# jstrom2002/Mini-OpenCL-Raytracer

Measured on AMD Instinct MI355X. Metric: Mrays/s (3840x2160 Cornell box, 8 spp, 9 bounces), higher is better.
Workload: dtype f32

## Files before the change

### include/rt_hip.h

```cpp
#ifndef RT_HIP_H
#define RT_HIP_H

#include <stddef.h>
#include <stdint.h>

#include "rt_cl_types.h"
#include "rt_status.h"

#ifdef __cplusplus
extern "C" {
#endif

typedef struct rt_context_s* rt_context;
typedef struct rt_mem_s* rt_mem;
typedef struct rt_kernel_s* rt_kernel;

#define RT_MEM_READ_WRITE (1u << 0)
#define RT_MEM_WRITE_ONLY (1u << 1)
#define RT_MEM_READ_ONLY (1u << 2)
#define RT_MEM_COPY_HOST_PTR (1u << 5)

enum rt_kernel_arg {
    RT_ARG_BUFFER_OUT = 0,
    RT_ARG_BUFFER_SCENE = 1,
// ... 68 lines not shown
    uint64_t launches;
    double kernel_ms;
    uint64_t cycles_refill, cycles_traverse, cycles_shade, cycles_total;
    uint64_t sched[12];
    double accum_ms;
    double render_period_ms;
} rt_stats;
int rtKernelSetStats(rt_kernel k, int enable);
int rtKernelSetTiming(rt_kernel k, int enable);
int rtKernelGetStats(rt_kernel k, rt_stats* out);
int rtKernelResetStats(rt_kernel k);

typedef struct rt_path_kill_info {
    uint64_t zero_hits, zero_misses;
    int32_t scene_certified, launch_certified;
} rt_path_kill_info;
int rtKernelGetPathKill(rt_kernel k, rt_path_kill_info* out);

typedef struct rt_node_collapse_info {
    uint32_t collapsed_links;
    int32_t scene_collapsible, launch_collapsed;
} rt_node_collapse_info;
int rtKernelGetNodeCollapse(rt_kernel k, rt_node_collapse_info* out);

typedef struct rt_ray {
    float origin[3];
    float tmin;
    float dir[3];
    float tmax;
} rt_ray;
typedef struct rt_ray_hit {
    int32_t prim;
    float t, u, v;
} rt_ray_hit;
#define RT_QUERY_CLOSEST 0
#define RT_QUERY_ANY 1
int rtEnqueueIntersectRays(rt_context ctx, rt_kernel k, rt_mem rays, size_t first_ray, size_t n_rays, int mode,
                           rt_mem hits);
int rtEnqueueCameraRays(rt_context ctx, rt_kernel k, size_t global_work_size, rt_mem rays);

typedef struct rt_path_result {
    float radiance[3];
    int32_t prim;
} rt_path_result;
#define RT_TRACE_LINEAR 0
#define RT_TRACE_FRAME0 1
// ... 232 lines not shown
```

### mini-opencl-raytracer_amd/clrt/_native.py

```python
from __future__ import annotations

import ctypes
import os

import numpy as np

_PKG_ROOT = os.path.dirname(os.path.dirname(os.path.abspath(__file__)))
LIB_DIR = os.path.join(_PKG_ROOT, "lib")
HIP_LIB_PATH = os.environ.get("RT_HIP_LIB") or os.path.join(LIB_DIR, "librt_hip.so")
SCENE_LIB_PATH = os.path.join(LIB_DIR, "librt_scene.so")

RT_SUCCESS = 0
_ERROR_NAMES = {
    0: "CL_SUCCESS", -1: "CL_DEVICE_NOT_FOUND", -4: "CL_MEM_OBJECT_ALLOCATION_FAILURE",
    -5: "CL_OUT_OF_RESOURCES", -6: "CL_OUT_OF_HOST_MEMORY", -30: "CL_INVALID_VALUE",
    -33: "CL_INVALID_DEVICE", -34: "CL_INVALID_CONTEXT", -36: "CL_INVALID_COMMAND_QUEUE",
    -37: "CL_INVALID_HOST_PTR", -38: "CL_INVALID_MEM_OBJECT", -46: "CL_INVALID_KERNEL_NAME",
    -48: "CL_INVALID_KERNEL", -49: "CL_INVALID_ARG_INDEX", -50: "CL_INVALID_ARG_VALUE",
    -51: "CL_INVALID_ARG_SIZE", -52: "CL_INVALID_KERNEL_ARGS", -59: "CL_INVALID_OPERATION",
    -61: "CL_INVALID_BUFFER_SIZE", -63: "CL_INVALID_GLOBAL_WORK_SIZE",
    -1001: "RT_FILE_NOT_FOUND", -1002: "RT_PARSE_ERROR",
}


# ... 69 lines not shown
          "step_weight_leaf_global": 25, "query_refill_min": 26}
TRACE_TUNING = {"trace_refill_min": 28, "trace_shade_min": 29}
PATH_KILL_TUNING = {"path_kill": 30}


class Stats(ctypes.Structure):
    _fields_ = [("rays", ctypes.c_uint64), ("node_visits", ctypes.c_uint64),
                ("tri_tests", ctypes.c_uint64), ("hits", ctypes.c_uint64),
                ("launches", ctypes.c_uint64), ("kernel_ms", ctypes.c_double),
                ("cycles_refill", ctypes.c_uint64), ("cycles_traverse", ctypes.c_uint64),
                ("cycles_shade", ctypes.c_uint64), ("cycles_total", ctypes.c_uint64),
                ("sched", ctypes.c_uint64 * 12), ("accum_ms", ctypes.c_double),
                ("render_period_ms", ctypes.c_double)]


class PathKillInfo(ctypes.Structure):
    _fields_ = [("zero_hits", ctypes.c_uint64), ("zero_misses", ctypes.c_uint64),
                ("scene_certified", ctypes.c_int32), ("launch_certified", ctypes.c_int32)]


class NodeCollapseInfo(ctypes.Structure):
    _fields_ = [("collapsed_links", ctypes.c_uint32), ("scene_collapsible", ctypes.c_int32),
                ("launch_collapsed", ctypes.c_int32)]


class TRACE_PARAMS(ctypes.Structure):
    _fields_ = [("seed_base", ctypes.c_uint32), ("encoding", ctypes.c_int)]


class ADAPTIVE_PARAMS(ctypes.Structure):
    _fields_ = [("threshold", ctypes.c_float), ("floor_y", ctypes.c_float), ("min_samples", ctypes.c_uint32),
                ("max_samples", ctypes.c_uint32), ("radius", ctypes.c_uint32)]


class DENOISE_PARAMS(ctypes.Structure):
    _fields_ = [("iterations", ctypes.c_uint), ("sigma_color", ctypes.c_float), ("sigma_normal", ctypes.c_float),
                ("sigma_depth", ctypes.c_float), ("sigma_albedo", ctypes.c_float)]


class DENOISE_SAMPLES_PARAMS(ctypes.Structure):
    _fields_ = [("iterations", ctypes.c_uint), ("sigma_luminance", ctypes.c_float), ("sigma_normal", ctypes.c_float),
                ("sigma_depth", ctypes.c_float), ("sigma_albedo", ctypes.c_float), ("epsilon", ctypes.c_float),
                ("encoding", ctypes.c_int)]


DENOISE_LINEAR, DENOISE_GAMMA = 0, 1
# ... 85 lines not shown
                                          ctypes.c_size_t, _vp]),
    "rtEnqueueFrameMotion": (ctypes.c_int, [_vp, _vp, ctypes.c_size_t, _vp, _vp, ctypes.c_size_t, ctypes.c_size_t, _vp]),
    "rtRefitBVH": (ctypes.c_int, [_vp, _vp]),
    "rtDiagScenePrepares": (ctypes.c_int, [_vp, ctypes.POINTER(ctypes.c_uint64), ctypes.POINTER(ctypes.c_uint64)]),
    "rtEnqueueReadBuffer": (ctypes.c_int, [_vp, _vp, ctypes.c_int, ctypes.c_size_t, ctypes.c_size_t, _vp]),
    "rtEnqueueWriteBuffer": (ctypes.c_int, [_vp, _vp, ctypes.c_int, ctypes.c_size_t, ctypes.c_size_t, _vp]),
    "rtFinish": (ctypes.c_int, [_vp]),
    "rtEnqueueCopyBufferToPointer": (ctypes.c_int, [_vp, _vp, ctypes.c_size_t, ctypes.c_size_t, _vp]),
    "rtKernelSetMathMode": (ctypes.c_int, [_vp, ctypes.c_int]),
    "rtKernelSetWorkRange": (ctypes.c_int, [_vp, ctypes.c_uint64, ctypes.c_uint64]),
    "rtKernelSetSchedule": (ctypes.c_int, [_vp, ctypes.c_int]),
    "rtKernelSetRowInterleave": (ctypes.c_int, [_vp, ctypes.c_uint, ctypes.c_uint]),
    "rtEnqueueCopyBufferRectToPointer": (ctypes.c_int, [_vp, _vp, ctypes.c_size_t, ctypes.c_size_t, ctypes.c_size_t,
                                                        ctypes.c_size_t, _vp, ctypes.c_size_t]),
    "rtEnqueueCopyPointerRectToBuffer": (ctypes.c_int, [_vp, _vp, ctypes.c_size_t, _vp, ctypes.c_size_t,
                                                        ctypes.c_size_t, ctypes.c_size_t, ctypes.c_size_t]),
    "rtKernelSetHitBuffers": (ctypes.c_int, [_vp, _vp, _vp]),
    "rtKernelSetStats": (ctypes.c_int, [_vp, ctypes.c_int]),
    "rtKernelSetTiming": (ctypes.c_int, [_vp, ctypes.c_int]),
    "rtKernelGetStats": (ctypes.c_int, [_vp, ctypes.POINTER(Stats)]),
    "rtKernelResetStats": (ctypes.c_int, [_vp]),
    "rtKernelGetPathKill": (ctypes.c_int, [_vp, ctypes.POINTER(PathKillInfo)]),
    "rtKernelGetNodeCollapse": (ctypes.c_int, [_vp, ctypes.POINTER(NodeCollapseInfo)]),
    "rtKernelGetSceneInLDS": (ctypes.c_int, [_vp, ctypes.POINTER(ctypes.c_int)]),
    "rtKernelForceGlobalScene": (ctypes.c_int, [_vp, ctypes.c_int]),
    "rtBuildBVH": (ctypes.c_int, [_vp, _vp, ctypes.c_size_t, ctypes.c_uint, _vp, ctypes.POINTER(ctypes.c_size_t)]),
    "rtBuildBVHEx": (ctypes.c_int, [_vp, _vp, ctypes.c_size_t, ctypes.c_uint, ctypes.c_int, _vp,
                                    ctypes.POINTER(ctypes.c_size_t)]),
    "rtBufferGetDevicePointer": (ctypes.c_int, [_vp, ctypes.POINTER(_vp)]),
    "rtBufferGetSize": (ctypes.c_int, [_vp, ctypes.POINTER(ctypes.c_size_t)]),
    "rtContextGetStream": (ctypes.c_int, [_vp, ctypes.POINTER(_vp)]),
    "rtContextSetReadbackOnAccumStream": (ctypes.c_int, [_vp, ctypes.c_int]),
    "rtContextGetAccumStream": (ctypes.c_int, [_vp, ctypes.POINTER(_vp)]),
    "rtContextGetDevice": (ctypes.c_int, [_vp, ctypes.POINTER(ctypes.c_int)]),
    "rtValidateBVH": (ctypes.c_int, [_vp, ctypes.c_size_t, ctypes.c_size_t, ctypes.POINTER(ctypes.c_int)]),
    "rtKernelSetTuning": (ctypes.c_int, [_vp, ctypes.c_int, ctypes.c_int]),
    "rtKernelGetTuning": (ctypes.c_int, [_vp, ctypes.c_int, ctypes.POINTER(ctypes.c_int)]),
    "rtContextSetAccumOverlap": (ctypes.c_int, [_vp, ctypes.c_int]),
    "rtCommGetUniqueId": (ctypes.c_int, [_vp]),
    "rtCommInitRank": (ctypes.c_int, [_vp, ctypes.c_int, _vp, ctypes.c_int, ctypes.POINTER(_vp)]),
    "rtCommInitAll": (ctypes.c_int, [ctypes.POINTER(_vp), ctypes.c_int, ctypes.POINTER(_vp)]),
    "rtCommInitLoopback": (ctypes.c_int, [ctypes.POINTER(_vp), ctypes.c_int, ctypes.POINTER(_vp)]),
    "rtCommInitShared": (ctypes.c_int, [_vp, ctypes.c_int, ctypes.c_int, ctypes.c_char_p, ctypes.POINTER(_vp)]),
    "rtCommDestroy": (ctypes.c_int, [_vp]),
    "rtCommGetRank": (ctypes.c_int, [_vp, ctypes.POINTER(ctypes.c_int), ctypes.POINTER(ctypes.c_int)]),
    "rtCommShardKernel": (ctypes.c_int, [_vp, _vp]),
# ... 80 lines not shown
```

### mini-opencl-raytracer_amd/clrt/device.py

```python
from __future__ import annotations

import ctypes
import struct

import numpy as np

from . import _native as N
from ._native import RTError, check, hip_lib


def _tuning_id(name: str) -> int:
    for table in (N.TUNING, N.TRACE_TUNING):
        if name in table:
            return table[name]
    return N.PATH_KILL_TUNING[name]


class CLContext:

    def __init__(self, device: int = 0):
        self._lib = hip_lib()
        h = ctypes.c_void_p()
        check(self._lib.rtCreateContext(int(device), ctypes.byref(h)), "Failed to create context")
        self.handle = h
# ... 331 lines not shown
        sched = dict(zip(("node_steps", "node_lanes", "tri_steps", "tri_lanes", "shade_rounds",
                          "shade_lanes", "refill_rounds", "refill_lanes", "other_lanes",
                          "shade_wait", "free_wait", "reserved"), list(s.sched)))
        sched["refill_pops"] = sched["reserved"]
        return {"rays": s.rays, "node_visits": s.node_visits, "tri_tests": s.tri_tests,
                "hits": s.hits, "launches": s.launches, "kernel_ms": s.kernel_ms, "accum_ms": s.accum_ms,
                "render_period_ms": s.render_period_ms,
                "cycles": {"refill": s.cycles_refill, "traverse": s.cycles_traverse,
                           "shade": s.cycles_shade, "total": s.cycles_total},
                "sched": sched}

    def path_kill(self) -> dict:
        s = N.PathKillInfo()
        check(self._lib.rtKernelGetPathKill(self.handle, ctypes.byref(s)), "path kill")
        return {"zero_hits": int(s.zero_hits), "zero_misses": int(s.zero_misses),
                "scene_certified": bool(s.scene_certified), "launch_certified": bool(s.launch_certified)}

    def node_collapse(self) -> dict:
        s = N.NodeCollapseInfo()
        check(self._lib.rtKernelGetNodeCollapse(self.handle, ctypes.byref(s)), "node collapse")
        return {"collapsed_links": int(s.collapsed_links), "scene_collapsible": bool(s.scene_collapsible),
                "launch_collapsed": bool(s.launch_collapsed)}

    def scene_prepares(self) -> tuple:
        full, refits = ctypes.c_uint64(), ctypes.c_uint64()
        check(self._lib.rtDiagScenePrepares(self.handle, ctypes.byref(full), ctypes.byref(refits)),
              "scene prepares")
        return int(full.value), int(refits.value)

    def reset_stats(self) -> None:
        check(self._lib.rtKernelResetStats(self.handle), "reset stats")

    def release(self) -> None:
        if self.handle:
            self._lib.rtReleaseKernel(self.handle)
            self.handle = None
```

### mini-opencl-raytracer_amd/csrc/rt_capi.cpp

```cpp
#include <hip/hip_runtime.h>

#include <algorithm>
#include <limits>
#include <cstdlib>
#include <cstring>
#include <mutex>
#include <new>
#include <vector>

#include "../../include/rt_cl_types.h"
#include "../../include/rt_hip.h"
#include "rt_adaptive.hpp"
#include "rt_adaptive_plan.hpp"
#include "rt_bvh.hpp"
#include "rt_denoise.hpp"
#include "rt_denoise_plan.hpp"
#include "rt_denoise_samples.hpp"
#include "rt_device_scene.hpp"
#include "rt_internal.hpp"
#include "rt_kernel_state.hpp"
#include "rt_kernels.hpp"
#include "rt_launch_plan.hpp"
#include "rt_motion_launch.hpp"
#include "rt_motion_plan.hpp"
#include "rt_query_plan.hpp"
#include "rt_refit.hpp"
#include "rt_reproject.hpp"
#include "rt_reproject_plan.hpp"
#include "rt_scene_pack.hpp"
#include "rt_temporal.hpp"
#include "rt_temporal_plan.hpp"
#include "rt_trace_plan.hpp"
#include "rt_tuning.hpp"

namespace {

constexpr uint64_t kKnownFlags =
    RT_MEM_READ_WRITE | RT_MEM_WRITE_ONLY | RT_MEM_READ_ONLY | RT_MEM_COPY_HOST_PTR;
#ifndef RT_TIMELINE
#define RT_TIMELINE 0
#endif
constexpr size_t kHitPad = RT_TIMELINE ? 192 : 0;
#ifndef RT_NODE_COLLAPSE_STATS
#define RT_NODE_COLLAPSE_STATS 0
#endif

}

using rti::map_hip;
using rti::mark_device_write;
using rti::qs;

struct rt_kernel_s {
    rt_context ctx = nullptr;
    rti::LaunchArgs args;
    int math = RT_MATH_SHIPPED;
    int sched = RT_SCHED_STEP;
    rtp::Tuning tune;
    uint32_t band_period = 1, band_phase = 0;
    uint64_t range_first = 0, range_last = 0;
    bool comm_sharded = false;
    rt_mem hit_ids = nullptr, hit_t = nullptr;
    bool stats = false, timing = false, force_global = false;
    uint64_t launches = 0;
    uint64_t pf_waits = ~0ull;
    bool last_lds = false;
    bool last_kill = false;
    bool last_collapsed = false;
    rti::DeviceScene scene;
    rti::LaunchTimer timer;
    rti::RadianceSets rad;
    rti::WavefrontQueues wfq;
    rti::WorkCounters counters;
    rti::FeatureScratch feat;
    rti::DenoiseScratch denoise;
    rti::AdaptiveScratch adaptive;
    rtk::OccupancyCache occ;

    void release_parts() {
        timer.release();
        rad.release();
        wfq.release();
        counters.release();
        scene.release();
        feat.release();
        denoise.release();
        adaptive.release();
    }
};

namespace {
// ... 334 lines not shown
    in.light_bounces = la.light_bounces();
    in.gws = global_work_size;
    in.range_first = k->range_first, in.range_last = k->range_last;
    in.n_frames = n_frames;
    in.sched = k->sched, in.math = k->math;
    in.stats = k->stats, in.hit_bound = k->hit_ids != nullptr;
    in.fused = fused, in.overlap = ctx->overlap;
    in.band_period = k->band_period, in.band_phase = k->band_phase;
    const rti::DeviceScene& sc = k->scene;
    in.n_nodes = sc.n_nodes(), in.n_tris = sc.n_tris(), in.n_mats = sc.n_mats(), in.n_top = sc.n_top();
    in.oct_ok = sc.oct_ok();
    in.goct_available = sc.goct() != nullptr, in.goct_b = sc.goct_b();
    in.force_global = k->force_global;
    in.tune = k->tune;
    in.num_cus = ctx->num_cus;
    if (const float* rb = sc.root_bounds()) in.view = rtp::view_cull_rect(in.W, in.H, la.f3[0], la.f3[1], la.f3[2], rb, rb + 3);
    in.kill_scene_ok = sc.path_kill_ok(k->math == RT_MATH_SHIPPED);
    in.light_type = la.light_type(), in.skybox_intensity = la.skybox_intensity();
    return in;
}

static const float4* oct_records(rt_kernel k, rtk::Walk w, bool regrouped) {
    const rti::DeviceScene& sc = k->scene;
    const bool collapsed = sc.collapse_ok() && (!k->stats || RT_NODE_COLLAPSE_STATS);
    k->last_collapsed = collapsed && w != rtk::Walk::GlobalNodes;
    if (collapsed) return regrouped ? sc.goct_collapsed() : sc.oct_nodes_collapsed();
    return regrouped ? sc.goct() : sc.oct_nodes();
}

static void fill_args(rt_kernel k, const LaunchArgs& la, uint32_t first_frame, const rtp::LaunchPlan& p,
                      rtk::KernelArgs* args) {
    rtk::KernelArgs& a = *args;
    std::memset(&a, 0, sizeof(a));
    a.result = static_cast<float4*>(la.out()->dptr);
    a.trisFull = static_cast<const rt_cl_triangle*>(la.tris()->dptr);
    a.materials = static_cast<const rt_cl_material*>(la.materials()->dptr);
    const rti::DeviceScene& sc = k->scene;
    a.packedTris = sc.packed_tris();
    a.octNodes = oct_records(k, p.variant.walk, p.regrouped);
    a.gNodes = sc.g_nodes();
    a.shadeTris = sc.shade_tris();
    a.shadeMats = sc.shade_mats() + (k->math == RT_MATH_SHIPPED ? 4 * (size_t)sc.n_mats() : 0);
    a.nMats = sc.n_mats(), a.nTris = sc.n_tris();
    a.nNodes = p.nNodes, a.octStride = p.octStride, a.octB = p.octB, a.octRecords = p.octRecords, a.nTop = p.nTop;
    fill_camera(la, first_frame, &a);
    a.lightBounces = la.light_bounces(), a.lightType = la.light_type();
    a.skyboxIntensity = la.skybox_intensity();
    a.gidBegin = p.gidBegin, a.gidEnd = p.gidEnd;
// ... 1144 lines not shown
    int rc = ensure_device(k->ctx);
    if (rc) return rc;
    unsigned long long h[2] = {};
    hipError_t e = hipMemcpyAsync(h, k->counters.stats() + rti::WorkCounters::kZeroBetaWord, sizeof(h),
                                  hipMemcpyDeviceToHost, qs(k->ctx));
    if (e == hipSuccess) e = hipStreamSynchronize(qs(k->ctx));
    if (e != hipSuccess) return map_hip(e);
    out->zero_hits = h[0];
    out->zero_misses = h[1];
    out->scene_certified = k->scene.path_kill_ok(k->math == RT_MATH_SHIPPED) ? 1 : 0;
    out->launch_certified = k->last_kill ? 1 : 0;
    return RT_SUCCESS;
}

int rtKernelGetNodeCollapse(rt_kernel k, rt_node_collapse_info* out) {
    if (!k || !out) return RT_INVALID_VALUE;
    flush_kernel(k);
    out->collapsed_links = k->scene.collapsed_links();
    out->scene_collapsible = k->scene.collapse_ok() ? 1 : 0;
    out->launch_collapsed = k->last_collapsed ? 1 : 0;
    return RT_SUCCESS;
}

int rtKernelResetStats(rt_kernel k) {
    if (!k) return RT_INVALID_KERNEL;
    flush_kernel(k);
    int rc = ensure_device(k->ctx);
    if (rc) return rc;
    rc = k->timer.drain();
    if (rc) return rc;
    k->launches = 0;
    k->timer.reset();
    hipError_t e = k->counters.zero_stats(qs(k->ctx));
    if (e == hipSuccess) e = hipStreamSynchronize(qs(k->ctx));
    return map_hip(e);
}

int rtKernelGetSceneInLDS(rt_kernel k, int* in_lds) {
    if (!k || !in_lds) return RT_INVALID_VALUE;
    *in_lds = k->last_lds ? 1 : 0;
    return RT_SUCCESS;
}

int rtKernelForceGlobalScene(rt_kernel k, int force) {
    if (!k) return RT_INVALID_KERNEL;
    flush_kernel(k);
// ... 104 lines not shown
```

### mini-opencl-raytracer_amd/csrc/rt_device_scene.cpp

```cpp
#include "rt_device_scene.hpp"

#include <cstring>
#include <vector>

#include "rt_kernels.hpp"
#include "rt_path_kill.hpp"
#include "rt_refit.hpp"
#include "rt_scene_pack.hpp"

namespace rti {

namespace {

int host_bytes(rt_mem m, std::vector<uint8_t>& tmp, const uint8_t** out) {
    if (m->shadow_valid) {
        *out = m->shadow.data();
        return RT_SUCCESS;
    }
    tmp.resize(m->size);
    hipError_t e = hipMemcpyAsync(tmp.data(), m->dptr, m->size, hipMemcpyDeviceToHost, qs(m->ctx));
    if (e == hipSuccess) e = hipStreamSynchronize(qs(m->ctx));
    if (e != hipSuccess) return map_hip(e);
    *out = tmp.data();
    return RT_SUCCESS;
}

template <class T>
int ensure_dev(T*& p, size_t& cap, size_t count) {
    if (cap >= count) return RT_SUCCESS;
    if (p) (void)hipFree(p);
    p = nullptr;
    cap = 0;
    hipError_t e = hipMalloc(&p, count * sizeof(T));
    if (e != hipSuccess) return map_hip(e);
    cap = count;
    return RT_SUCCESS;
}

hipError_t upload(void* dst, const std::vector<uint32_t>& src, hipStream_t st) {
    return hipMemcpyAsync(dst, src.data(), src.size() * sizeof(uint32_t), hipMemcpyHostToDevice, st);
}

}

int DeviceScene::allocate(uint32_t nn, uint32_t nt, uint32_t nmat, size_t goct_words, bool collapsed) {
    int rc = ensure_dev(g_nodes_, g_nodes_cap_, (size_t)nn * 4);
    if (!rc) rc = ensure_dev(refit_links_, refit_links_cap_, (size_t)nn * 2);
    if (!rc) rc = ensure_dev(refit_arrivals_, refit_arrivals_cap_, (size_t)nn);
    if (!rc) rc = ensure_dev(oct_nodes_, oct_nodes_cap_, (size_t)rtp::oct_records(nn));
    if (!rc) rc = ensure_dev(goct_nodes_, goct_nodes_cap_, goct_words / 4);
    if (!rc && collapsed) rc = ensure_dev(oct_collapsed_, oct_collapsed_cap_, (size_t)rtp::oct_records(nn));
    if (!rc && collapsed) rc = ensure_dev(goct_collapsed_, goct_collapsed_cap_, goct_words / 4);
    if (!rc) rc = ensure_dev(packed_tris_, packed_tris_cap_, (size_t)nt * 3);
    if (!rc) rc = ensure_dev(shade_tris_, shade_tris_cap_, (size_t)nt * 3);
    if (!rc) rc = ensure_dev(shade_mats_, shade_mats_cap_, (size_t)nmat * 8);
    return rc;
}

int DeviceScene::prepare(rt_context ctx, rt_mem tm, rt_mem nm, rt_mem mm) {
    if (!stale(tm, nm, mm)) return RT_SUCCESS;
    std::vector<uint8_t> tmp_t, tmp_n;
    rtp::SceneBytes in;
    in.tris_size = tm->size, in.nodes_size = nm->size;
    int rc = host_bytes(tm, tmp_t, &in.tris);
    if (!rc) rc = host_bytes(nm, tmp_n, &in.nodes);
    if (rc) return rc;
    if (mm) {
        in.mats = static_cast<const uint8_t*>(mm->dptr);
        in.mats_size = mm->size;
    }
    rtp::HostPack p;
    rc = rtp::pack_scene_host(in, top_limit, &p);
    if (rc) return rc;
    invalidate();
    rc = allocate(p.n_nodes, p.n_tris, p.n_mats, p.goct_nodes.size(), p.collapsed_links != 0);
    if (rc) return rc;
    hipStream_t st = qs(ctx);
    hipError_t e = upload(g_nodes_, p.global_nodes, st);
    if (e == hipSuccess) e = upload(refit_links_, p.refit_links, st);
    if (e == hipSuccess) e = upload(oct_nodes_, p.oct_nodes, st);
    if (e == hipSuccess && !p.goct_nodes.empty()) e = upload(goct_nodes_, p.goct_nodes, st);
    if (e == hipSuccess && p.collapsed_links) e = upload(oct_collapsed_, p.oct_nodes_collapsed, st);
    if (e == hipSuccess && !p.goct_nodes_collapsed.empty()) e = upload(goct_collapsed_, p.goct_nodes_collapsed, st);
    if (e == hipSuccess)
        e = rtk::launch_pack(static_cast<const rt_cl_triangle*>(tm->dptr), p.n_tris, packed_tris_, shade_tris_,
                             mm ? static_cast<const rt_cl_material*>(mm->dptr) : nullptr, p.n_mats, shade_mats_, st);
    const hipError_t waited = hipStreamSynchronize(st);
    if (e == hipSuccess) e = waited;
    if (e != hipSuccess) return map_hip(e);
    n_nodes_ = p.n_nodes, n_tris_ = p.n_tris, n_mats_ = p.n_mats, n_top_ = p.n_top;
    oct_ok_ = p.oct_ok, goct_b_ = p.goct_b;
    collapsed_links_ = p.collapsed_links, collapse_known_ = RT_NODE_COLLAPSE != 0;
    root_known_ = p.n_nodes > 0 && in.nodes_size >= sizeof(rt_cl_bvh_node);
    if (root_known_) {
        rt_cl_bvh_node root;
        std::memcpy(&root, in.nodes, sizeof(root));
        const float b[6] = {root.bounds.pmin.x, root.bounds.pmin.y, root.bounds.pmin.z,
                            root.bounds.pmax.x, root.bounds.pmax.y, root.bounds.pmax.z};
        std::memcpy(root_bounds_, b, sizeof(b));
    }
    kill_known_ = false;
    if (mm && p.n_mats > 0) {
        std::vector<float> recs((size_t)p.n_mats * 32);
        e = hipMemcpyAsync(recs.data(), shade_mats_, recs.size() * sizeof(float), hipMemcpyDeviceToHost, st);
        if (e == hipSuccess) e = hipStreamSynchronize(st);
        if (e != hipSuccess) return map_hip(e);
        const rt_cl_triangle* ht = reinterpret_cast<const rt_cl_triangle*>(in.tris);
        for (int t = 0; t < 2; ++t)
            kill_ok_[t] = rtp::path_kill_scene_ok(recs.data() + (size_t)t * 16 * p.n_mats, p.n_mats, ht, p.n_tris,
                                                  root_bounds());
        kill_known_ = true;
    }
    for_tris_ = tm, tris_gen_ = tm->generation, tris_struct_ = tm->structural;
    for_nodes_ = nm, nodes_gen_ = nm->generation, nodes_struct_ = nm->structural;
    for_mats_ = mm, mats_gen_ = mm ? mm->generation : 0;
// ... 2 lines not shown
}

int DeviceScene::refit(rt_context ctx, rt_mem tm, rt_mem nm, rt_mem mm) {
    if (!structurally_current(tm, nm)) {
        invalidate();
        const int rc = prepare(ctx, tm, nm, mm);
        if (rc) return rc;
    }
    rtr::RefitArgs a{};
    a.tris = static_cast<const rt_cl_triangle*>(tm->dptr);
    a.n_tris = n_tris_;
    a.nodes = static_cast<rt_cl_bvh_node*>(nm->dptr);
    a.n_nodes = n_nodes_;
    a.parent = refit_links_;
    a.slot = refit_links_ + n_nodes_;
    a.arrivals = refit_arrivals_;
    a.oct = oct_nodes_;
    a.oct_stride = rtp::oct_stride(n_nodes_), a.oct_b = rtp::oct_b(n_nodes_);
    a.goct = goct_b_ ? goct_nodes_ : nullptr;
    a.goct_b = goct_b_, a.goct_group = RT_GOCT_GROUP ? RT_GOCT_GROUP : 1;
    a.g_nodes = g_nodes_;
    root_known_ = false;
    collapse_known_ = false;
    kill_known_ = false;
    hipStream_t st = qs(ctx);
    hipError_t e = rtr::launch_refit(a, st);
    if (e == hipSuccess) e = rtk::launch_pack(a.tris, n_tris_, packed_tris_, shade_tris_, nullptr, 0, shade_mats_, st);
    mark_device_write(nm, false);
    if (e != hipSuccess) {
        invalidate();
        return map_hip(e);
    }
    tris_gen_ = tm->generation;
    nodes_gen_ = nm->generation;
    ++refits_;
    return RT_SUCCESS;
}

void DeviceScene::release() {
    for (void* p : {(void*)packed_tris_, (void*)shade_tris_, (void*)shade_mats_, (void*)oct_nodes_, (void*)goct_nodes_,
                    (void*)oct_collapsed_, (void*)goct_collapsed_, (void*)g_nodes_, (void*)refit_links_,
                    (void*)refit_arrivals_})
        if (p) (void)hipFree(p);
    *this = DeviceScene();
}

}
```

### mini-opencl-raytracer_amd/csrc/rt_device_scene.hpp

```cpp
#pragma once

#include <hip/hip_runtime.h>
#include <stdint.h>

#include "rt_internal.hpp"

namespace rti {

class DeviceScene {
public:
    uint32_t top_limit = 384;

    int prepare(rt_context ctx, rt_mem tris, rt_mem nodes, rt_mem mats);
    int refit(rt_context ctx, rt_mem tris, rt_mem nodes, rt_mem mats);
    void invalidate() { for_nodes_ = nullptr; }
    void release();

    uint32_t n_nodes() const { return n_nodes_; }
    uint32_t n_tris() const { return n_tris_; }
    uint32_t n_mats() const { return n_mats_; }
    uint32_t n_top() const { return n_top_; }
    bool oct_ok() const { return oct_ok_; }
    uint32_t goct_b() const { return goct_b_; }
    const float4* packed_tris() const { return packed_tris_; }
    const float4* shade_tris() const { return shade_tris_; }
    const float4* shade_mats() const { return shade_mats_; }
    const float4* oct_nodes() const { return oct_nodes_; }
    const float4* g_nodes() const { return g_nodes_; }
    const float4* goct() const { return goct_b_ ? goct_nodes_ : nullptr; }
    bool collapse_ok() const { return collapse_known_; }
    uint32_t collapsed_links() const { return collapsed_links_; }
    const float4* oct_nodes_collapsed() const { return collapsed_links_ ? oct_collapsed_ : oct_nodes_; }
    const float4* goct_collapsed() const { return collapsed_links_ && goct_b_ ? goct_collapsed_ : goct(); }
    const float* root_bounds() const { return root_known_ ? root_bounds_ : nullptr; }
    bool path_kill_ok(bool shipped) const { return kill_known_ && kill_ok_[shipped ? 1 : 0]; }
    uint64_t full_prepares() const { return full_prepares_; }
    uint64_t refits() const { return refits_; }

private:
    bool stale(rt_mem tris, rt_mem nodes, rt_mem mats) const {
        return for_tris_ != tris || tris_gen_ != tris->generation || for_nodes_ != nodes ||
               nodes_gen_ != nodes->generation || (mats && (for_mats_ != mats || mats_gen_ != mats->generation));
    }
    bool structurally_current(rt_mem tris, rt_mem nodes) const {
        return for_tris_ == tris && for_nodes_ == nodes && tris_struct_ == tris->structural &&
               nodes_struct_ == nodes->structural;
    }
    int allocate(uint32_t n_nodes, uint32_t n_tris, uint32_t n_mats, size_t goct_words, bool collapsed);

    rt_mem for_tris_ = nullptr, for_nodes_ = nullptr, for_mats_ = nullptr;
    uint64_t tris_gen_ = 0, nodes_gen_ = 0, mats_gen_ = 0;
    uint64_t tris_struct_ = 0, nodes_struct_ = 0;
    uint32_t n_nodes_ = 0, n_tris_ = 0, n_mats_ = 0, n_top_ = 0, goct_b_ = 0;
    bool oct_ok_ = false;
    bool root_known_ = false;
    float root_bounds_[6] = {};
    bool collapse_known_ = false;
    uint32_t collapsed_links_ = 0;
    bool kill_known_ = false;
    bool kill_ok_[2] = {false, false};
    uint64_t full_prepares_ = 0, refits_ = 0;
    float4 *packed_tris_ = nullptr, *shade_tris_ = nullptr, *shade_mats_ = nullptr;
    float4 *oct_nodes_ = nullptr, *goct_nodes_ = nullptr, *g_nodes_ = nullptr;
    size_t packed_tris_cap_ = 0, shade_tris_cap_ = 0, shade_mats_cap_ = 0;
    size_t oct_nodes_cap_ = 0, goct_nodes_cap_ = 0, g_nodes_cap_ = 0;
    float4 *oct_collapsed_ = nullptr, *goct_collapsed_ = nullptr;
    size_t oct_collapsed_cap_ = 0, goct_collapsed_cap_ = 0;
    uint32_t *refit_links_ = nullptr, *refit_arrivals_ = nullptr;
    size_t refit_links_cap_ = 0, refit_arrivals_cap_ = 0;
};

}
```

### mini-opencl-raytracer_amd/csrc/rt_scene_pack.cpp

```cpp
#include "rt_scene_pack.hpp"

#include <algorithm>
#include <cstring>
#include <limits>

#include "../../include/rt_status.h"

namespace rtp {

int check_nodes(const rt_cl_bvh_node* nd, uint32_t n, uint32_t n_tris, int* depth_out, uint32_t* n_used) {
    if (n == 0) return RT_INVALID_MEM_OBJECT;
    uint32_t last = 0;
    while (nd[last].nPrimitives == 0) {
        if (nd[last].offset <= last || nd[last].offset >= n) return RT_INVALID_MEM_OBJECT;
        last = nd[last].offset;
    }
    n = last + 1;
    std::vector<int> depth(n, -1);
    std::vector<uint8_t> parents(n, 0);
    depth[0] = 0;
    int max_depth = 0;
    for (uint32_t i = 0; i < n; ++i) {
        const rt_cl_bvh_node& x = nd[i];
        if (i > 0 && parents[i] != 1) return RT_INVALID_MEM_OBJECT;
// ... 83 lines not shown
}

uint32_t collapse_oct_links(const std::vector<uint32_t>& oct, uint32_t n, std::vector<uint32_t>& out) {
    const uint32_t stride = oct_stride(n), bofs = oct_b(n);
    out = oct;
    uint32_t changed = 0;
    for (uint32_t o = 0; o < 8; ++o) {
        const uint32_t* pa = &oct[(size_t)o * stride * 4];
        const uint32_t* pb = &oct[((size_t)bofs + (size_t)o * stride) * 4];
        auto same_box = [&](uint32_t x, uint32_t y) {
            return std::memcmp(pa + (size_t)x * 4, pa + (size_t)y * 4, 16) == 0 &&
                   std::memcmp(pb + (size_t)x * 4, pb + (size_t)y * 4, 8) == 0;
        };
        for (uint32_t i = 0; i < n; ++i) {
            const uint32_t near0 = pb[(size_t)i * 4 + 2];
            if (near0 >= kLeafMin) continue;
            uint32_t c = near0;
            while (pb[(size_t)c * 4 + 2] < kLeafMin && same_box(i, c)) c = pb[(size_t)c * 4 + 2];
            if (c != near0) {
                out[((size_t)bofs + (size_t)o * stride + i) * 4 + 2] = c;
                ++changed;
            }
        }
    }
    return changed;
}

void build_oct_nodes_grouped(const std::vector<uint32_t>& oct, uint32_t n, uint32_t G, std::vector<uint32_t>& out,
                             uint32_t* b_ofs) {
    const uint32_t stride = oct_stride(n), bofs = oct_b(n);
    const uint32_t na = ((n + 1 + G - 1) / G) * 8u * G;
    *b_ofs = na;
    out.assign((size_t)2 * na * 4, 0u);
    for (uint32_t i = 0; i <= n; ++i)
        for (uint32_t o = 0; o < 8; ++o) {
            const uint32_t* ra = &oct[((size_t)o * stride + i) * 4];
            const uint32_t* rb = &oct[((size_t)bofs + (size_t)o * stride + i) * 4];
            const size_t at = (size_t)goct_word(i, G) + (size_t)o * G;
            uint32_t* wa = &out[at * 4];
            uint32_t* wb = &out[((size_t)na + at) * 4];
            for (int c = 0; c < 4; ++c) wa[c] = ra[c];
            wb[0] = rb[0];
            wb[1] = rb[1];
            wb[2] = rb[2] >= kLeafMin ? rb[2] : goct_word(rb[2], G);
            wb[3] = rb[3] >= n && RT_GOCT_END_WORD ? rtk::kEndWalk : goct_word(rb[3], G);
        }
// ... 76 lines not shown
    for (uint32_t i = 0; in.mats && i < p.n_tris; ++i)
        if (tr[i].mtlIndex >= p.n_mats) return RT_INVALID_MEM_OBJECT;
    const uint32_t nn = p.n_nodes;
    if (nn >= (1u << 30)) return RT_INVALID_MEM_OBJECT;
    std::vector<uint32_t> skips, slot_of;
    build_skips(nd, nn, skips);
    build_global_nodes(nd, nn, skips, top_limit, p.global_nodes, &p.n_top, &slot_of);
    build_refit_links(nd, nn, slot_of, p.refit_links);
    p.oct_ok = build_oct_nodes(nd, nn, skips, p.oct_nodes);
    if (RT_GOCT_GROUP && p.oct_ok && (uint64_t)(nn + RT_GOCT_GROUP) * 8u < kLeafMin)
        build_oct_nodes_grouped(p.oct_nodes, nn, RT_GOCT_GROUP, p.goct_nodes, &p.goct_b);
    if (RT_NODE_COLLAPSE && p.oct_ok) {
        p.collapsed_links = collapse_oct_links(p.oct_nodes, nn, p.oct_nodes_collapsed);
        if (p.collapsed_links == 0) {
            p.oct_nodes_collapsed.clear();
        } else if (!p.goct_nodes.empty()) {
            uint32_t b = 0;
            build_oct_nodes_grouped(p.oct_nodes_collapsed, nn, RT_GOCT_GROUP, p.goct_nodes_collapsed, &b);
        }
    }
    return RT_SUCCESS;
}

}
```

### mini-opencl-raytracer_amd/csrc/rt_scene_pack.hpp

```cpp
#pragma once

#include <stddef.h>
#include <stdint.h>

#include <vector>

#include "../../include/rt_cl_types.h"
#include "rt_layout.hpp"

namespace rtp {

constexpr uint32_t kLeafMin = 1u << 24;

inline uint32_t oct_stride(uint32_t n) { return (n + 1) | 1u; }
inline uint32_t oct_b(uint32_t n) {
    return oct_stride(n) <= rtk::kOctBMaxStride ? rtk::kOctB : 8u * oct_stride(n);
}
inline uint32_t oct_records(uint32_t n) { return oct_b(n) + 8u * oct_stride(n); }

#ifndef RT_NODE_COLLAPSE
#define RT_NODE_COLLAPSE 1
#endif
#ifndef RT_GOCT_GROUP
#define RT_GOCT_GROUP 1
#endif
inline uint32_t goct_word(uint32_t i, uint32_t G) { return (i / G) * 8u * G + i % G; }

int check_nodes(const rt_cl_bvh_node* nd, uint32_t n, uint32_t n_tris, int* depth_out, uint32_t* n_used);
void build_skips(const rt_cl_bvh_node* nd, uint32_t n, std::vector<uint32_t>& skips);
bool build_oct_nodes(const rt_cl_bvh_node* nd, uint32_t n, const std::vector<uint32_t>& skips,
                     std::vector<uint32_t>& out);
void build_oct_nodes_grouped(const std::vector<uint32_t>& oct, uint32_t n, uint32_t G, std::vector<uint32_t>& out,
                             uint32_t* b_ofs);
uint32_t collapse_oct_links(const std::vector<uint32_t>& oct, uint32_t n, std::vector<uint32_t>& out);
void build_global_nodes(const rt_cl_bvh_node* nd, uint32_t n, const std::vector<uint32_t>& skips,
                        uint32_t top, std::vector<uint32_t>& out, uint32_t* n_top,
                        std::vector<uint32_t>* slot_of = nullptr);
void build_refit_links(const rt_cl_bvh_node* nd, uint32_t n, const std::vector<uint32_t>& slot_of,
                       std::vector<uint32_t>& out);

struct SceneBytes {
    const uint8_t* tris = nullptr;
    size_t tris_size = 0;
    const uint8_t* nodes = nullptr;
    size_t nodes_size = 0;
    const uint8_t* mats = nullptr;
    size_t mats_size = 0;
};

struct HostPack {
    uint32_t n_nodes = 0, n_tris = 0, n_mats = 0;
    int depth = 0;
    uint32_t n_top = 0;
    bool oct_ok = false;
    uint32_t goct_b = 0;
    std::vector<uint32_t> global_nodes, refit_links, oct_nodes;
    std::vector<uint32_t> goct_nodes;
    uint32_t collapsed_links = 0;
    std::vector<uint32_t> oct_nodes_collapsed, goct_nodes_collapsed;
};

int pack_scene_host(const SceneBytes& in, uint32_t top_limit, HostPack* out);

}
```

Baseline: 48920.

## Prune BVH links to subtrees whose triangles all backface-cull for a ray octant

On the host, each triangle gets a mask of the ray-direction octants for which it always faces away from the ray (sign of the normal components, computed with a conservative margin). Per-octant oct-node planes then rewrite child and skip links to jump over subtrees made entirely of such triangles, and a pruned node buffer is uploaded and selected by default. This cuts node visits and triangle tests for rays that could never hit those triangles. It relies on the intersection kernel already culling backfaces; if it does not, closest hits could be lost. It also adds extra device buffers and host preprocessing at scene build.

```diff
diff --git a/include/rt_hip.h b/include/rt_hip.h
--- a/include/rt_hip.h
+++ b/include/rt_hip.h
@@ -114,6 +114,12 @@
     int32_t scene_collapsible, launch_collapsed;
 } rt_node_collapse_info;
 int rtKernelGetNodeCollapse(rt_kernel k, rt_node_collapse_info* out);
+
+typedef struct rt_octant_cull_info {
+    uint32_t pruned_links, contracted_links;
+    int32_t scene_certified, launch_pruned;
+} rt_octant_cull_info;
+int rtKernelGetOctantCull(rt_kernel k, rt_octant_cull_info* out);
 
 typedef struct rt_ray {
     float origin[3];
diff --git a/mini-opencl-raytracer_amd/clrt/_native.py b/mini-opencl-raytracer_amd/clrt/_native.py
--- a/mini-opencl-raytracer_amd/clrt/_native.py
+++ b/mini-opencl-raytracer_amd/clrt/_native.py
@@ -115,6 +115,11 @@
 class NodeCollapseInfo(ctypes.Structure):
     _fields_ = [("collapsed_links", ctypes.c_uint32), ("scene_collapsible", ctypes.c_int32),
                 ("launch_collapsed", ctypes.c_int32)]
+
+
+class OctantCullInfo(ctypes.Structure):
+    _fields_ = [("pruned_links", ctypes.c_uint32), ("contracted_links", ctypes.c_uint32),
+                ("scene_certified", ctypes.c_int32), ("launch_pruned", ctypes.c_int32)]
 
 
 class TRACE_PARAMS(ctypes.Structure):
@@ -246,6 +251,7 @@
     "rtKernelResetStats": (ctypes.c_int, [_vp]),
     "rtKernelGetPathKill": (ctypes.c_int, [_vp, ctypes.POINTER(PathKillInfo)]),
     "rtKernelGetNodeCollapse": (ctypes.c_int, [_vp, ctypes.POINTER(NodeCollapseInfo)]),
+    "rtKernelGetOctantCull": (ctypes.c_int, [_vp, ctypes.POINTER(OctantCullInfo)]),
     "rtKernelGetSceneInLDS": (ctypes.c_int, [_vp, ctypes.POINTER(ctypes.c_int)]),
     "rtKernelForceGlobalScene": (ctypes.c_int, [_vp, ctypes.c_int]),
     "rtBuildBVH": (ctypes.c_int, [_vp, _vp, ctypes.c_size_t, ctypes.c_uint, _vp, ctypes.POINTER(ctypes.c_size_t)]),
diff --git a/mini-opencl-raytracer_amd/clrt/device.py b/mini-opencl-raytracer_amd/clrt/device.py
--- a/mini-opencl-raytracer_amd/clrt/device.py
+++ b/mini-opencl-raytracer_amd/clrt/device.py
@@ -377,6 +377,12 @@
         return {"collapsed_links": int(s.collapsed_links), "scene_collapsible": bool(s.scene_collapsible),
                 "launch_collapsed": bool(s.launch_collapsed)}
 
+    def octant_cull(self) -> dict:
+        s = N.OctantCullInfo()
+        check(self._lib.rtKernelGetOctantCull(self.handle, ctypes.byref(s)), "octant cull")
+        return {"pruned_links": int(s.pruned_links), "contracted_links": int(s.contracted_links),
+                "scene_certified": bool(s.scene_certified), "launch_pruned": bool(s.launch_pruned)}
+
     def scene_prepares(self) -> tuple:
         full, refits = ctypes.c_uint64(), ctypes.c_uint64()
         check(self._lib.rtDiagScenePrepares(self.handle, ctypes.byref(full), ctypes.byref(refits)),
diff --git a/mini-opencl-raytracer_amd/csrc/rt_capi.cpp b/mini-opencl-raytracer_amd/csrc/rt_capi.cpp
--- a/mini-opencl-raytracer_amd/csrc/rt_capi.cpp
+++ b/mini-opencl-raytracer_amd/csrc/rt_capi.cpp
@@ -44,6 +44,9 @@
 #ifndef RT_NODE_COLLAPSE_STATS
 #define RT_NODE_COLLAPSE_STATS 0
 #endif
+#ifndef RT_OCTANT_CULL_STATS
+#define RT_OCTANT_CULL_STATS 0
+#endif
 
 }
 
@@ -67,6 +70,7 @@
     bool last_lds = false;
     bool last_kill = false;
     bool last_collapsed = false;
+    bool last_pruned = false;
     rti::DeviceScene scene;
     rti::LaunchTimer timer;
     rti::RadianceSets rad;
@@ -447,8 +451,11 @@
 
 static const float4* oct_records(rt_kernel k, rtk::Walk w, bool regrouped) {
     const rti::DeviceScene& sc = k->scene;
-    const bool collapsed = sc.collapse_ok() && (!k->stats || RT_NODE_COLLAPSE_STATS);
+    const bool pruned = sc.cull_ok() && (!k->stats || RT_OCTANT_CULL_STATS);
+    const bool collapsed = sc.collapse_ok() && (!k->stats || RT_NODE_COLLAPSE_STATS || pruned);
     k->last_collapsed = collapsed && w != rtk::Walk::GlobalNodes;
+    k->last_pruned = pruned && w != rtk::Walk::GlobalNodes;
+    if (pruned) return regrouped ? sc.goct_pruned() : sc.oct_nodes_pruned();
     if (collapsed) return regrouped ? sc.goct_collapsed() : sc.oct_nodes_collapsed();
     return regrouped ? sc.goct() : sc.oct_nodes();
 }
@@ -1639,6 +1646,16 @@
     return RT_SUCCESS;
 }
 
+int rtKernelGetOctantCull(rt_kernel k, rt_octant_cull_info* out) {
+    if (!k || !out) return RT_INVALID_VALUE;
+    flush_kernel(k);
+    out->pruned_links = k->scene.pruned_links();
+    out->contracted_links = 0;
+    out->scene_certified = k->scene.cull_ok() ? 1 : 0;
+    out->launch_pruned = k->last_pruned ? 1 : 0;
+    return RT_SUCCESS;
+}
+
 int rtKernelResetStats(rt_kernel k) {
     if (!k) return RT_INVALID_KERNEL;
     flush_kernel(k);
diff --git a/mini-opencl-raytracer_amd/csrc/rt_device_scene.cpp b/mini-opencl-raytracer_amd/csrc/rt_device_scene.cpp
--- a/mini-opencl-raytracer_amd/csrc/rt_device_scene.cpp
+++ b/mini-opencl-raytracer_amd/csrc/rt_device_scene.cpp
@@ -4,6 +4,7 @@
 #include <vector>
 
 #include "rt_kernels.hpp"
+#include "rt_octant_cull.hpp"
 #include "rt_path_kill.hpp"
 #include "rt_refit.hpp"
 #include "rt_scene_pack.hpp"
@@ -43,7 +44,8 @@
 
 }
 
-int DeviceScene::allocate(uint32_t nn, uint32_t nt, uint32_t nmat, size_t goct_words, bool collapsed) {
+int DeviceScene::allocate(uint32_t nn, uint32_t nt, uint32_t nmat, size_t goct_words, bool collapsed,
+                          bool pruned) {
     int rc = ensure_dev(g_nodes_, g_nodes_cap_, (size_t)nn * 4);
     if (!rc) rc = ensure_dev(refit_links_, refit_links_cap_, (size_t)nn * 2);
     if (!rc) rc = ensure_dev(refit_arrivals_, refit_arrivals_cap_, (size_t)nn);
@@ -51,6 +53,8 @@
     if (!rc) rc = ensure_dev(goct_nodes_, goct_nodes_cap_, goct_words / 4);
     if (!rc && collapsed) rc = ensure_dev(oct_collapsed_, oct_collapsed_cap_, (size_t)rtp::oct_records(nn));
     if (!rc && collapsed) rc = ensure_dev(goct_collapsed_, goct_collapsed_cap_, goct_words / 4);
+    if (!rc && pruned) rc = ensure_dev(oct_pruned_, oct_pruned_cap_, (size_t)rtp::oct_records(nn));
+    if (!rc && pruned) rc = ensure_dev(goct_pruned_, goct_pruned_cap_, goct_words / 4);
     if (!rc) rc = ensure_dev(packed_tris_, packed_tris_cap_, (size_t)nt * 3);
     if (!rc) rc = ensure_dev(shade_tris_, shade_tris_cap_, (size_t)nt * 3);
     if (!rc) rc = ensure_dev(shade_mats_, shade_mats_cap_, (size_t)nmat * 8);
@@ -72,8 +76,14 @@
     rtp::HostPack p;
     rc = rtp::pack_scene_host(in, top_limit, &p);
     if (rc) return rc;
+    if (RT_OCTANT_CULL && p.oct_ok) {
+        std::vector<uint8_t> tri_octants(p.n_tris);
+        rtp::octant_cull_masks(reinterpret_cast<const rt_cl_triangle*>(in.tris), p.n_tris, tri_octants.data());
+        rtp::pack_pruned_links(tri_octants.data(), &p);
+    }
     invalidate();
-    rc = allocate(p.n_nodes, p.n_tris, p.n_mats, p.goct_nodes.size(), p.collapsed_links != 0);
+    rc = allocate(p.n_nodes, p.n_tris, p.n_mats, p.goct_nodes.size(), p.collapsed_links != 0,
+                  p.pruned_links != 0);
     if (rc) return rc;
     hipStream_t st = qs(ctx);
     hipError_t e = upload(g_nodes_, p.global_nodes, st);
@@ -82,6 +92,8 @@
     if (e == hipSuccess && !p.goct_nodes.empty()) e = upload(goct_nodes_, p.goct_nodes, st);
     if (e == hipSuccess && p.collapsed_links) e = upload(oct_collapsed_, p.oct_nodes_collapsed, st);
     if (e == hipSuccess && !p.goct_nodes_collapsed.empty()) e = upload(goct_collapsed_, p.goct_nodes_collapsed, st);
+    if (e == hipSuccess && p.pruned_links) e = upload(oct_pruned_, p.oct_nodes_pruned, st);
+    if (e == hipSuccess && !p.goct_nodes_pruned.empty()) e = upload(goct_pruned_, p.goct_nodes_pruned, st);
     if (e == hipSuccess)
         e = rtk::launch_pack(static_cast<const rt_cl_triangle*>(tm->dptr), p.n_tris, packed_tris_, shade_tris_,
                              mm ? static_cast<const rt_cl_material*>(mm->dptr) : nullptr, p.n_mats, shade_mats_, st);
@@ -91,6 +103,7 @@
     n_nodes_ = p.n_nodes, n_tris_ = p.n_tris, n_mats_ = p.n_mats, n_top_ = p.n_top;
     oct_ok_ = p.oct_ok, goct_b_ = p.goct_b;
     collapsed_links_ = p.collapsed_links, collapse_known_ = RT_NODE_COLLAPSE != 0;
+    pruned_links_ = p.pruned_links, cull_known_ = RT_OCTANT_CULL != 0 && p.oct_ok;
     root_known_ = p.n_nodes > 0 && in.nodes_size >= sizeof(rt_cl_bvh_node);
     if (root_known_) {
         rt_cl_bvh_node root;
@@ -139,6 +152,7 @@
     a.g_nodes = g_nodes_;
     root_known_ = false;
     collapse_known_ = false;
+    cull_known_ = false;
     kill_known_ = false;
     hipStream_t st = qs(ctx);
     hipError_t e = rtr::launch_refit(a, st);
@@ -156,7 +170,8 @@
 
 void DeviceScene::release() {
     for (void* p : {(void*)packed_tris_, (void*)shade_tris_, (void*)shade_mats_, (void*)oct_nodes_, (void*)goct_nodes_,
-                    (void*)oct_collapsed_, (void*)goct_collapsed_, (void*)g_nodes_, (void*)refit_links_,
+                    (void*)oct_collapsed_, (void*)goct_collapsed_, (void*)oct_pruned_, (void*)goct_pruned_,
+                    (void*)g_nodes_, (void*)refit_links_,
                     (void*)refit_arrivals_})
         if (p) (void)hipFree(p);
     *this = DeviceScene();
diff --git a/mini-opencl-raytracer_amd/csrc/rt_device_scene.hpp b/mini-opencl-raytracer_amd/csrc/rt_device_scene.hpp
--- a/mini-opencl-raytracer_amd/csrc/rt_device_scene.hpp
+++ b/mini-opencl-raytracer_amd/csrc/rt_device_scene.hpp
@@ -32,6 +32,10 @@
     uint32_t collapsed_links() const { return collapsed_links_; }
     const float4* oct_nodes_collapsed() const { return collapsed_links_ ? oct_collapsed_ : oct_nodes_; }
     const float4* goct_collapsed() const { return collapsed_links_ && goct_b_ ? goct_collapsed_ : goct(); }
+    bool cull_ok() const { return cull_known_; }
+    uint32_t pruned_links() const { return pruned_links_; }
+    const float4* oct_nodes_pruned() const { return pruned_links_ ? oct_pruned_ : oct_nodes_collapsed(); }
+    const float4* goct_pruned() const { return pruned_links_ && goct_b_ ? goct_pruned_ : goct_collapsed(); }
     const float* root_bounds() const { return root_known_ ? root_bounds_ : nullptr; }
     bool path_kill_ok(bool shipped) const { return kill_known_ && kill_ok_[shipped ? 1 : 0]; }
     uint64_t full_prepares() const { return full_prepares_; }
@@ -46,7 +50,7 @@
         return for_tris_ == tris && for_nodes_ == nodes && tris_struct_ == tris->structural &&
                nodes_struct_ == nodes->structural;
     }
-    int allocate(uint32_t n_nodes, uint32_t n_tris, uint32_t n_mats, size_t goct_words, bool collapsed);
+    int allocate(uint32_t n_nodes, uint32_t n_tris, uint32_t n_mats, size_t goct_words, bool collapsed, bool pruned);
 
     rt_mem for_tris_ = nullptr, for_nodes_ = nullptr, for_mats_ = nullptr;
     uint64_t tris_gen_ = 0, nodes_gen_ = 0, mats_gen_ = 0;
@@ -57,6 +61,8 @@
     float root_bounds_[6] = {};
     bool collapse_known_ = false;
     uint32_t collapsed_links_ = 0;
+    bool cull_known_ = false;
+    uint32_t pruned_links_ = 0;
     bool kill_known_ = false;
     bool kill_ok_[2] = {false, false};
     uint64_t full_prepares_ = 0, refits_ = 0;
@@ -66,6 +72,8 @@
     size_t oct_nodes_cap_ = 0, goct_nodes_cap_ = 0, g_nodes_cap_ = 0;
     float4 *oct_collapsed_ = nullptr, *goct_collapsed_ = nullptr;
     size_t oct_collapsed_cap_ = 0, goct_collapsed_cap_ = 0;
+    float4 *oct_pruned_ = nullptr, *goct_pruned_ = nullptr;
+    size_t oct_pruned_cap_ = 0, goct_pruned_cap_ = 0;
     uint32_t *refit_links_ = nullptr, *refit_arrivals_ = nullptr;
     size_t refit_links_cap_ = 0, refit_arrivals_cap_ = 0;
 };
diff --git a/mini-opencl-raytracer_amd/csrc/rt_octant_cull.cpp b/mini-opencl-raytracer_amd/csrc/rt_octant_cull.cpp
--- /dev/null
+++ b/mini-opencl-raytracer_amd/csrc/rt_octant_cull.cpp
@@ -0,0 +1,60 @@
+#include "rt_octant_cull.hpp"
+
+#include <cmath>
+
+namespace rtp {
+
+namespace {
+
+constexpr float kCoordMax = 0x1p20f;
+constexpr double kMargin = 0x1p-18;
+
+bool coord_ok(const rt_float3& p) {
+    return std::isfinite(p.x) && std::isfinite(p.y) && std::isfinite(p.z) && std::fabs(p.x) <= kCoordMax &&
+           std::fabs(p.y) <= kCoordMax && std::fabs(p.z) <= kCoordMax;
+}
+
+}
+
+CullEdges octant_cull_edges(const rt_cl_triangle& t) {
+    const rt_float3 &p1 = t.v1.position, &p2 = t.v2.position, &p3 = t.v3.position;
+    return CullEdges{{p2.x - p1.x, p2.y - p1.y, p2.z - p1.z}, {p3.x - p1.x, p3.y - p1.y, p3.z - p1.z}};
+}
+
+uint8_t octant_cull_mask(const rt_cl_triangle& t) {
+    if (!coord_ok(t.v1.position) || !coord_ok(t.v2.position) || !coord_ok(t.v3.position)) return 0;
+    const CullEdges e = octant_cull_edges(t);
+    int sign[3];
+    for (int k = 0; k < 3; ++k) {
+        const int i = (k + 2) % 3, j = (k + 1) % 3;
+        const double a = (double)e.e1[i] * e.e2[j], b = (double)e.e1[j] * e.e2[i];
+        const double c = a - b;
+        if (a == 0.0 && b == 0.0)
+            sign[k] = 0;
+        else if (c != 0.0 && std::fabs(c) >= kMargin * (std::fabs(a) + std::fabs(b)))
+            sign[k] = c < 0.0 ? -1 : 1;
+        else
+            return 0;
+    }
+    uint8_t mask = 0;
+    for (uint32_t o = 0; o < 8; ++o) {
+        bool ok = true;
+        for (int k = 0; k < 3; ++k) {
+            const int s = ((o >> k) & 1u) ? -1 : 1;
+            ok = ok && (sign[k] == 0 || s * sign[k] < 0);
+        }
+        if (ok) mask |= (uint8_t)(1u << o);
+    }
+    return mask;
+}
+
+uint32_t octant_cull_masks(const rt_cl_triangle* tris, uint32_t n_tris, uint8_t* mask) {
+    uint32_t pairs = 0;
+    for (uint32_t i = 0; i < n_tris; ++i) {
+        mask[i] = octant_cull_mask(tris[i]);
+        pairs += (uint32_t)__builtin_popcount(mask[i]);
+    }
+    return pairs;
+}
+
+}
diff --git a/mini-opencl-raytracer_amd/csrc/rt_octant_cull.hpp b/mini-opencl-raytracer_amd/csrc/rt_octant_cull.hpp
--- /dev/null
+++ b/mini-opencl-raytracer_amd/csrc/rt_octant_cull.hpp
@@ -0,0 +1,18 @@
+#pragma once
+
+#include <stdint.h>
+
+#include "../../include/rt_cl_types.h"
+
+namespace rtp {
+
+struct CullEdges {
+    float e1[3], e2[3];
+};
+CullEdges octant_cull_edges(const rt_cl_triangle& t);
+
+uint8_t octant_cull_mask(const rt_cl_triangle& t);
+
+uint32_t octant_cull_masks(const rt_cl_triangle* tris, uint32_t n_tris, uint8_t* mask);
+
+}
diff --git a/mini-opencl-raytracer_amd/csrc/rt_scene_pack.cpp b/mini-opencl-raytracer_amd/csrc/rt_scene_pack.cpp
--- a/mini-opencl-raytracer_amd/csrc/rt_scene_pack.cpp
+++ b/mini-opencl-raytracer_amd/csrc/rt_scene_pack.cpp
@@ -129,6 +129,46 @@
                 ++changed;
             }
         }
+    }
+    return changed;
+}
+
+uint32_t prune_oct_links(const std::vector<uint32_t>& oct, const std::vector<uint32_t>& base, uint32_t n,
+                         const uint8_t* tri_octants, std::vector<uint32_t>& out) {
+    const uint32_t stride = oct_stride(n), bofs = oct_b(n);
+    out = base;
+    uint32_t changed = 0;
+    std::vector<uint8_t> culled(n);
+    for (uint32_t o = 0; o < 8; ++o) {
+        const size_t plane = ((size_t)bofs + (size_t)o * stride) * 4;
+        const uint32_t* pb = &oct[plane];
+        for (uint32_t i = n; i-- > 0;) {
+            const uint32_t hn = pb[(size_t)i * 4 + 2];
+            if (hn >= kLeafMin) {
+                const uint32_t first = hn & (kLeafMin - 1), count = hn >> 24;
+                bool all = true;
+                for (uint32_t t = first; t < first + count; ++t) all = all && ((tri_octants[t] >> o) & 1u);
+                culled[i] = all;
+            } else {
+                const uint32_t farc = pb[(size_t)hn * 4 + 3];
+                culled[i] = culled[hn] && farc < n && culled[farc];
+            }
+        }
+        if (culled[0]) continue;
+        auto live = [&](uint32_t x) {
+            while (x < n && culled[x]) x = pb[(size_t)x * 4 + 3];
+            return x;
+        };
+        for (uint32_t i = 0; i < n; ++i)
+            for (uint32_t k = 2; k < 4; ++k) {
+                uint32_t& w = out[plane + (size_t)i * 4 + k];
+                if (w >= kLeafMin) continue;
+                const uint32_t to = live(w);
+                if (to != w) {
+                    w = to;
+                    ++changed;
+                }
+            }
     }
     return changed;
 }
@@ -251,4 +291,20 @@
     return RT_SUCCESS;
 }
 
-}
+void pack_pruned_links(const uint8_t* tri_octants, HostPack* pack) {
+    HostPack& p = *pack;
+    p.pruned_links = 0;
+    p.oct_nodes_pruned.clear();
+    p.goct_nodes_pruned.clear();
+    if (!RT_OCTANT_CULL || !p.oct_ok || !tri_octants) return;
+    const std::vector<uint32_t>& base = p.collapsed_links ? p.oct_nodes_collapsed : p.oct_nodes;
+    p.pruned_links = prune_oct_links(p.oct_nodes, base, p.n_nodes, tri_octants, p.oct_nodes_pruned);
+    if (p.pruned_links == 0) {
+        p.oct_nodes_pruned.clear();
+    } else if (!p.goct_nodes.empty()) {
+        uint32_t b = 0;
+        build_oct_nodes_grouped(p.oct_nodes_pruned, p.n_nodes, RT_GOCT_GROUP, p.goct_nodes_pruned, &b);
+    }
+}
+
+}
diff --git a/mini-opencl-raytracer_amd/csrc/rt_scene_pack.hpp b/mini-opencl-raytracer_amd/csrc/rt_scene_pack.hpp
--- a/mini-opencl-raytracer_amd/csrc/rt_scene_pack.hpp
+++ b/mini-opencl-raytracer_amd/csrc/rt_scene_pack.hpp
@@ -21,6 +21,9 @@
 #ifndef RT_NODE_COLLAPSE
 #define RT_NODE_COLLAPSE 1
 #endif
+#ifndef RT_OCTANT_CULL
+#define RT_OCTANT_CULL 1
+#endif
 #ifndef RT_GOCT_GROUP
 #define RT_GOCT_GROUP 1
 #endif
@@ -33,6 +36,8 @@
 void build_oct_nodes_grouped(const std::vector<uint32_t>& oct, uint32_t n, uint32_t G, std::vector<uint32_t>& out,
                              uint32_t* b_ofs);
 uint32_t collapse_oct_links(const std::vector<uint32_t>& oct, uint32_t n, std::vector<uint32_t>& out);
+uint32_t prune_oct_links(const std::vector<uint32_t>& oct, const std::vector<uint32_t>& base, uint32_t n,
+                         const uint8_t* tri_octants, std::vector<uint32_t>& out);
 void build_global_nodes(const rt_cl_bvh_node* nd, uint32_t n, const std::vector<uint32_t>& skips,
                         uint32_t top, std::vector<uint32_t>& out, uint32_t* n_top,
                         std::vector<uint32_t>* slot_of = nullptr);
@@ -58,8 +63,11 @@
     std::vector<uint32_t> goct_nodes;
     uint32_t collapsed_links = 0;
     std::vector<uint32_t> oct_nodes_collapsed, goct_nodes_collapsed;
+    uint32_t pruned_links = 0;
+    std::vector<uint32_t> oct_nodes_pruned, goct_nodes_pruned;
 };
 
 int pack_scene_host(const SceneBytes& in, uint32_t top_limit, HostPack* out);
+void pack_pruned_links(const uint8_t* tri_octants, HostPack* pack);
 
 }
```

New measurement: 49680 (median of 6 runs). 1.02x the previous value.
